# LouisNUST/pose-unsupervised

Measured on AMD Instinct MI355X. Metric: 4-view 256x256 frames/sec (fwd+triangulate), higher is better.
Workload: dtype bf16

## Files before the change

### pose-unsupervised_amd/csrc/stem.hip

```cpp
#include <string>
#include <type_traits>

#include "posu_common.h"

namespace posu {
namespace {

constexpr int kStemK = 224;
constexpr int kStemPitch = 232;
typedef unsigned int u32x4 __attribute__((ext_vector_type(4)));

template <typename T>
struct StemOp;
template <>
struct StemOp<uint16_t> {
  static __device__ __forceinline__ void mma(f32x4& acc, const uint4& a, const uint4& b) {
    acc = __builtin_amdgcn_mfma_f32_16x16x32_bf16(__builtin_bit_cast(bf16x8, a), __builtin_bit_cast(bf16x8, b), acc,
                                                  0, 0, 0);
  }
  static __device__ __forceinline__ uint32_t pack2(float a, float b) {
    return f2bf2(a, b);
  }
};
template <>
struct StemOp<f16_t> {
  static __device__ __forceinline__ void mma(f32x4& acc, const uint4& a, const uint4& b) {
    acc = __builtin_amdgcn_mfma_f32_16x16x32_f16(__builtin_bit_cast(f16x8, a), __builtin_bit_cast(f16x8, b), acc, 0,
                                                 0, 0);
  }
  static __device__ __forceinline__ uint32_t pack2(float a, float b) {
    const _Float16 ha = static_cast<_Float16>(a), hb = static_cast<_Float16>(b);
    return static_cast<uint32_t>(__builtin_bit_cast(uint16_t, ha)) |
           (static_cast<uint32_t>(__builtin_bit_cast(uint16_t, hb)) << 16);
  }
};

constexpr int kMaxViews = 8;
struct StemViews {
  const float* x[kMaxViews];
};

#ifndef POSU_STEM_ABLATE
#define POSU_STEM_ABLATE 0
#endif
#ifndef POSU_STEM_PFD
#define POSU_STEM_PFD 1
#endif
constexpr int kStemAbl = POSU_STEM_ABLATE;

template <typename T, int NW, bool SPL = false, bool RAW = false>
__global__ __launch_bounds__(NW * 64, 1) void stem_pool_kernel(StemViews xs, int Nv, int N, int H, int W, int hflip,
                                                               int strips, const void* __restrict__ wv_,
                                                               const float* __restrict__ scale,
                                                               const float* __restrict__ shift, T* __restrict__ y) {
  using O = StemOp<T>;
  constexpr int NT = NW * 64;
  constexpr int WP = NW * 32 + 8;
  constexpr int RB = WP * 8;
  constexpr int RING = 16;
  constexpr int W_BYTES = 64 * kStemPitch * 2;
  constexpr int NS = SPL ? 2 : 1;
  constexpr int CPX = SPL ? 128 : 64;
  static_assert(!SPL || (NW == 8 && std::is_same<T, f16_t>::value), "split stem: fp16 halves, eight waves");
  static_assert(!RAW || (!SPL && NW == 8), "raw stem: one dtype, eight waves");
  const T* __restrict__ w = static_cast<const T*>(wv_);
  __shared__ __attribute__((aligned(16))) char smem[NS * (RING * RB + W_BYTES) + NW * 2 * 64 * 4 + 2 * 64 * 4];
  char* win = smem;
  char* winl = smem + RING * RB;
  char* wl = smem + NS * RING * RB;
  char* wll = wl + W_BYTES;
  float* edge = reinterpret_cast<float*>(smem + NS * (RING * RB + W_BYTES));
  float* bn = edge + NW * 2 * 64;

  const int tid = threadIdx.x, lane = tid & 63, wid = tid >> 6;
  const int r16 = lane & 15, q = lane >> 4;
  const int Hp = H / 4, Wp = W / 4;
  const int pairs = Hp / 2, per = pairs / strips;
  const int n = blockIdx.x / strips;
  const int k0 = (blockIdx.x - n * strips) * per, k1 = k0 + per;
  const float* __restrict__ xn = xs.x[n / Nv] + static_cast<size_t>(n % Nv) * 3 * H * W;
  const size_t plane = static_cast<size_t>(H) * W;

  if constexpr (RAW) {
    const float* __restrict__ wf = static_cast<const float*>(wv_);
    for (int i = tid; i < 64 * kStemK / 2; i += NT) {
      const int co = i / (kStemK / 2), k0 = 2 * (i - co * (kStemK / 2));
      float v[2];
#pragma unroll
      for (int u = 0; u < 2; ++u) {
        const int k = k0 + u, kh = k >> 5, kw = (k >> 2) & 7, ci = k & 3;
        v[u] = (kw < 7 && ci < 3) ? wf[((co * 3 + ci) * 7 + kh) * 7 + kw] : 0.f;
      }
      *reinterpret_cast<uint32_t*>(wl + (co * kStemPitch + k0) * 2) = O::pack2(v[0], v[1]);
    }
  } else {
  if (tid < 64) {
    bn[tid] = fabsf(scale[tid]);
    bn[64 + tid] = shift[tid];
  }
  {
    constexpr int WCH = 64 * (kStemK / 8);
#pragma unroll
    for (int it = 0; it < (NS * WCH + NT - 1) / NT; ++it) {
      const int i = tid + it * NT;
      if (i < NS * WCH) {
        const int h = i / WCH, ii = i - h * WCH;
        const int co = ii / (kStemK / 8), ck = ii - co * (kStemK / 8);
        const unsigned sg = __float_as_uint(scale[co]) & 0x80000000u ? 0x80008000u : 0u;
        u32x4 wv = *reinterpret_cast<const u32x4*>(w + i * 8);
        wv ^= sg;
        *reinterpret_cast<u32x4*>((h ? wll : wl) + (co * kStemPitch + ck * 8) * 2) = wv;
      }
    }
  }
  }

  constexpr int GPR = NW * 8 + 2;
  constexpr int XG8 = (8 * GPR + NT - 1) / NT;
  auto load_rows = [&](int i0, auto nr, float4 (*xv)[3]) __attribute__((always_inline)) {
    constexpr int NR = decltype(nr)::value, XG = (NR * GPR + NT - 1) / NT;
#pragma unroll
    for (int it = 0; it < XG; ++it) {
      const int i = tid + it * NT;
      const int r = i / GPR, gk = i - r * GPR;
      const int iy = i0 + r, c0 = 4 * (gk - 1);
#pragma unroll
      for (int p = 0; p < 3; ++p) xv[it][p] = make_float4(0.f, 0.f, 0.f, 0.f);
      if (kStemAbl & 2) {
        xv[it][0] = make_float4(iy, c0, 1.f, 0.5f);
        continue;
      }
      if (i < NR * GPR && static_cast<unsigned>(iy) < static_cast<unsigned>(H) &&
          static_cast<unsigned>(c0) < static_cast<unsigned>(W)) {
        const size_t o = static_cast<size_t>(iy) * W + (hflip ? W - 4 - c0 : c0);
#pragma unroll
        for (int p = 0; p < 3; ++p) {
          float4 v = *reinterpret_cast<const float4*>(xn + p * plane + o);
          if (hflip) v = make_float4(v.w, v.z, v.y, v.x);
          xv[it][p] = v;
        }
      }
    }
  };
  auto store_rows = [&](int i0, auto nr, float4 (*xv)[3]) __attribute__((always_inline)) {
    constexpr int NR = decltype(nr)::value, XG = (NR * GPR + NT - 1) / NT;
#pragma unroll
    for (int it = 0; it < XG; ++it) {
      const int i = tid + it * NT;
      if (i >= NR * GPR) continue;
      const int r = i / GPR, gk = i - r * GPR;
      char* row = win + ((i0 + r) & (RING - 1)) * RB;
      const float a0[4] = {xv[it][0].x, xv[it][0].y, xv[it][0].z, xv[it][0].w};
      const float a1[4] = {xv[it][1].x, xv[it][1].y, xv[it][1].z, xv[it][1].w};
      const float a2[4] = {xv[it][2].x, xv[it][2].y, xv[it][2].z, xv[it][2].w};
#pragma unroll
      for (int e = 0; e < 4; ++e) {
        const int wc = 4 * gk - 1 + e;
        if (wc >= 0 && wc < WP) {
          *reinterpret_cast<uint2*>(row + wc * 8) = make_uint2(O::pack2(a0[e], a1[e]), O::pack2(a2[e], 0.f));
          if constexpr (SPL) {
            const float l0 = a0[e] - static_cast<float>(static_cast<_Float16>(a0[e]));
            const float l1 = a1[e] - static_cast<float>(static_cast<_Float16>(a1[e]));
            const float l2 = a2[e] - static_cast<float>(static_cast<_Float16>(a2[e]));
            *reinterpret_cast<uint2*>(row - win + winl + wc * 8) = make_uint2(O::pack2(l0, l1), O::pack2(l2, 0.f));
          }
        }
      }
    }
  };

  const int sc = 16 * wid + r16;
  auto stem_rows = [&](int r0, auto mrows, float (*carry)[4], float (*vm)[4][4]) __attribute__((always_inline)) {
    constexpr int M = decltype(mrows)::value;
    f32x4 acc[M][4];
#pragma unroll
    for (int i = 0; i < M; ++i)
#pragma unroll
      for (int j = 0; j < 4; ++j) acc[i][j] = f32x4{0.f, 0.f, 0.f, 0.f};
    auto rd = [&](int rho) {
      return *reinterpret_cast<const uint4*>(win + ((2 * r0 - 3 + rho) & (RING - 1)) * RB + (2 * sc + 2 * q) * 8);
    };
    auto rdl = [&](int rho) {
      return *reinterpret_cast<const uint4*>(winl + ((2 * r0 - 3 + rho) & (RING - 1)) * RB + (2 * sc + 2 * q) * 8);
    };
    auto bload = [&](int kh, uint4 (&bfr)[4]) {
#pragma unroll
      for (int j = 0; j < 4; ++j)
        bfr[j] = *reinterpret_cast<const uint4*>(wl + ((16 * j + r16) * kStemPitch + kh * 32 + 8 * q) * 2);
    };
    auto bloadl = [&](int kh, uint4 (&bfr)[4]) {
#pragma unroll
      for (int j = 0; j < 4; ++j)
        bfr[j] = *reinterpret_cast<const uint4*>(wll + ((16 * j + r16) * kStemPitch + kh * 32 + 8 * q) * 2);
    };
    auto mmas = [&](const uint4 (&bfr)[4], const uint4 (&af)[M]) {
#pragma unroll
      for (int rl = 0; rl < M; ++rl)
#pragma unroll
        for (int j = 0; j < 4; ++j) {
          if (kStemAbl & 1) acc[rl][j][0] += __uint_as_float(bfr[j].x ^ af[rl].y);
          else O::mma(acc[rl][j], bfr[j], af[rl]);
        }
    };
    if constexpr (SPL) {
      uint4 ev[M], od[M], evl[M], odl[M], bfr[4], bfl[4];
#pragma unroll
      for (int kh = 0; kh < 7; ++kh) {
        uint4 (&set)[M] = (kh & 1) ? od : ev;
        uint4 (&setl)[M] = (kh & 1) ? odl : evl;
        bload(kh, bfr);
        bloadl(kh, bfl);
        if (kh < 2) {
#pragma unroll
          for (int rl = 0; rl < M; ++rl) {
            set[rl] = rd(kh + 2 * rl);
            setl[rl] = rdl(kh + 2 * rl);
          }
        } else {
#pragma unroll
          for (int rl = 0; rl + 1 < M; ++rl) {
            set[rl] = set[rl + 1];
            setl[rl] = setl[rl + 1];
          }
          set[M - 1] = rd(kh + 2 * (M - 1));
          setl[M - 1] = rdl(kh + 2 * (M - 1));
        }
        mmas(bfr, set);
        mmas(bfl, set);
        mmas(bfr, setl);
      }
    } else if constexpr (NW <= 8) {
      uint4 ev[M], od[M], bfr[4];
#pragma unroll
      for (int kh = 0; kh < 7; ++kh) {
        uint4 (&set)[M] = (kh & 1) ? od : ev;
        bload(kh, bfr);
        if (kh < 2) {
#pragma unroll
          for (int rl = 0; rl < M; ++rl) set[rl] = rd(kh + 2 * rl);
        } else {
#pragma unroll
          for (int rl = 0; rl + 1 < M; ++rl) set[rl] = set[rl + 1];
          set[M - 1] = rd(kh + 2 * (M - 1));
        }
        mmas(bfr, set);
      }
    } else {
#pragma unroll 1
      for (int kh = 0; kh < 7; ++kh) {
        uint4 bfr[4];
        bload(kh, bfr);
#pragma unroll
        for (int rl = 0; rl < M; ++rl) {
          const uint4 af = rd(kh + 2 * rl);
#pragma unroll
          for (int j = 0; j < 4; ++j) O::mma(acc[rl][j], bfr[j], af);
        }
      }
    }
    if constexpr (RAW) {
      T* __restrict__ zr = y + (static_cast<size_t>(n) * (H / 2) + r0) * (W / 2) * 64 + sc * 64 + 4 * q;
#pragma unroll
      for (int rl = 0; rl < M; ++rl)
#pragma unroll
        for (int j = 0; j < 4; ++j) {
          const uint2 u = make_uint2(O::pack2(acc[rl][j][0], acc[rl][j][1]), O::pack2(acc[rl][j][2], acc[rl][j][3]));
          if (kStemAbl & 4) asm volatile("" ::"v"(u.x), "v"(u.y));
          else *reinterpret_cast<uint2*>(zr + static_cast<size_t>(rl) * (W / 2) * 64 + 16 * j) = u;
        }
      return;
    }
#pragma unroll
    for (int j = 0; j < 4; ++j)
#pragma unroll
      for (int e = 0; e < 4; ++e) {
        float v[M];
#pragma unroll
        for (int rl = 0; rl < M; ++rl)
          v[rl] = (M == 4 || r0 + rl >= 0) ? acc[rl][j][e] : -INFINITY;
        const float first = M == 5 ? v[0] : carry[j][e];
        const float* u = v + (M == 5 ? 1 : 0);
        vm[0][j][e] = fmaxf(fmaxf(first, u[0]), u[1]);
        vm[1][j][e] = fmaxf(fmaxf(u[1], u[2]), u[3]);
        carry[j][e] = u[3];
      }
  };

  T* __restrict__ yn = y + static_cast<size_t>(n) * Hp * Wp * CPX;
  auto pool = [&](int k, const float (*vm)[4][4]) __attribute__((always_inline)) {
    if (r16 == 15) {
#pragma unroll
      for (int p = 0; p < 2; ++p)
#pragma unroll
        for (int j = 0; j < 4; ++j)
          *reinterpret_cast<float4*>(edge + (wid * 2 + p) * 64 + 16 * j + 4 * q) =
              make_float4(vm[p][j][0], vm[p][j][1], vm[p][j][2], vm[p][j][3]);
    }
    __syncthreads();
    const int wl = wid > 0 ? wid - 1 : 0;
    const bool first_col = r16 == 0, pad_left = wid == 0;
#pragma unroll
    for (int p = 0; p < 2; ++p)
#pragma unroll
      for (int j = 0; j < 4; ++j) {
        const float4 s4 = *reinterpret_cast<const float4*>(bn + 16 * j + 4 * q);
        const float4 b4 = *reinterpret_cast<const float4*>(bn + 64 + 16 * j + 4 * q);
        const float sv[4] = {s4.x, s4.y, s4.z, s4.w}, bv[4] = {b4.x, b4.y, b4.z, b4.w};
        const float4 l4 = *reinterpret_cast<const float4*>(edge + (wl * 2 + p) * 64 + 16 * j + 4 * q);
        const float lv[4] = {l4.x, l4.y, l4.z, l4.w};
        float o[4];
#pragma unroll
        for (int e = 0; e < 4; ++e) {
          const float self = vm[p][j][e];
          const float right = __int_as_float(__builtin_amdgcn_update_dpp(0, __float_as_int(self), 0x101, 0xf, 0xf, true));
          float left = __int_as_float(__builtin_amdgcn_update_dpp(0, __float_as_int(self), 0x111, 0xf, 0xf, true));
          if (first_col) left = pad_left ? -INFINITY : lv[e];
          o[e] = fmaxf(fmaf(sv[e], fmaxf(fmaxf(left, self), right), bv[e]), 0.f);
        }
        if ((r16 & 1) == 0) {
          const int pc = 8 * wid + (r16 >> 1);
          const int c0 = 16 * j + 4 * q;
          T* dst = yn + (static_cast<size_t>(2 * k + p) * Wp + pc) * CPX + (SPL ? split_ch(c0) : c0);
          const uint2 u = make_uint2(O::pack2(o[0], o[1]), O::pack2(o[2], o[3]));
          if (kStemAbl & 4) {
            asm volatile("" ::"v"(u.x), "v"(u.y));
          } else {
            *reinterpret_cast<uint2*>(dst) = u;
            if constexpr (SPL) {
              float l[4];
#pragma unroll
              for (int e = 0; e < 4; ++e) l[e] = o[e] - static_cast<float>(static_cast<_Float16>(o[e]));
              *reinterpret_cast<uint2*>(dst + 32) = make_uint2(O::pack2(l[0], l[1]), O::pack2(l[2], l[3]));
            }
          }
        }
      }
  };

  using I4 = std::integral_constant<int, 4>;
  using I5 = std::integral_constant<int, 5>;
  using I8 = std::integral_constant<int, 8>;
  float carry[4][4], vm[2][4][4];
  constexpr bool PF = NW <= 8;
  constexpr int PFD = PF ? POSU_STEM_PFD : 1;
  static_assert(PFD == 1 || PFD == 2, "prefetch depth 1 or 2");
  float4 xv[PFD][XG8][3];
  load_rows(8 * k0 - 5, I8{}, xv[0]);
  store_rows(8 * k0 - 5, I8{}, xv[0]);
  load_rows(8 * k0 + 3, I8{}, xv[0]);
  store_rows(8 * k0 + 3, I8{}, xv[0]);
  __syncthreads();
  if constexpr (RAW) stem_rows(4 * k0, I4{}, carry, vm);
  else stem_rows(4 * k0 - 1, I5{}, carry, vm);
  if constexpr (PF) {
    if (k0 + 1 < k1) load_rows(8 * k0 + 10, I8{}, xv[PFD - 1]);
    if (PFD == 2 && k0 + 2 < k1) load_rows(8 * k0 + 18, I8{}, xv[0]);
  }
  if constexpr (RAW) __syncthreads();
  else pool(k0, vm);
  auto item = [&](int k, auto sidx) __attribute__((always_inline)) {
    constexpr int S = decltype(sidx)::value;
    if (!PF) load_rows(8 * k + 2, I8{}, xv[S]);
    store_rows(8 * k + 2, I8{}, xv[S]);
    __syncthreads();
    if (PF && k + PFD < k1) load_rows(8 * (k + PFD) + 2, I8{}, xv[S]);
    if constexpr (PF) stem_rows(4 * k, I4{}, carry, vm);
    else stem_rows(4 * k - 1, I5{}, carry, vm);
    if constexpr (RAW) {
      __syncthreads();
    } else {
      pool(k, vm);
    }
  };
  using S0 = std::integral_constant<int, 0>;
  using S1 = std::integral_constant<int, PFD - 1>;
  int k = k0 + 1;
  if constexpr (PFD == 2) {
    for (; k + 1 < k1; k += 2) {
      item(k, S1{});
      item(k + 1, S0{});
    }
  }
  for (; k < k1; ++k) item(k, S1{});
}


typedef short s16x4 __attribute__((ext_vector_type(4)));
constexpr int kWgThreads = 448;
constexpr int kWgRing = 16;
constexpr int kWgCols = 264;
constexpr int kWgRB = kWgCols * 8;
constexpr int kWgDz = 128 * 128;
constexpr int kWgGroups = 66;
constexpr int kWgPart = 7 * 32 * 64;

__device__ __forceinline__ int wg_sw(int px) { return (((px >> 1) & 1) << 1) | (((px >> 3) & 1) << 2); }

__device__ __forceinline__ uint4 tr_pair(const char* p0, const char* p1) {
  const s16x4 v0 = __builtin_amdgcn_ds_read_tr16_b64_v4i16((__attribute__((address_space(3))) s16x4*)(p0));
  const s16x4 v1 = __builtin_amdgcn_ds_read_tr16_b64_v4i16((__attribute__((address_space(3))) s16x4*)(p1));
  const uint2 u0 = __builtin_bit_cast(uint2, v0), u1 = __builtin_bit_cast(uint2, v1);
  return make_uint4(u0.x, u0.y, u1.x, u1.y);
}

template <typename T>
__global__ __launch_bounds__(kWgThreads, 2) void stem_wgrad_kernel(StemViews xs, int Nv, int H, int strips,
                                                                   const T* __restrict__ dz, float* __restrict__ part) {
  using O = StemOp<T>;
  constexpr int W = 256, Wo = 128;
  __shared__ __attribute__((aligned(16))) char smem[kWgRing * kWgRB + 2 * kWgDz];
  char* ring = smem;
  char* dzb = smem + kWgRing * kWgRB;
  const int tid = threadIdx.x, lane = tid & 63, kh = tid >> 6;
  const int q = lane >> 4, a = (lane >> 2) & 3, p = lane & 3;
  const int Ho = H / 2, rows = Ho / strips;
  const int n = blockIdx.x / strips;
  const int ya = (blockIdx.x - n * strips) * rows, yb = ya + rows;
  const float* __restrict__ xn = xs.x[n / Nv] + static_cast<size_t>(n % Nv) * 3 * H * W;
  const size_t plane = static_cast<size_t>(H) * W;
  const T* __restrict__ dzn = dz + static_cast<size_t>(n) * Ho * Wo * 64;

  auto load_x = [&](int iy0, int nr, int it, float4 (&xv)[3]) {
    const int i = tid + it * kWgThreads;
    const int r = i / kWgGroups, g = i - r * kWgGroups;
    const int iy = iy0 + r, c0 = 4 * (g - 1);
    const bool ok = i < nr * kWgGroups && static_cast<unsigned>(iy) < static_cast<unsigned>(H) &&
                    static_cast<unsigned>(c0) < static_cast<unsigned>(W);
    const size_t o = ok ? static_cast<size_t>(iy) * W + c0 : 0;
#pragma unroll
    for (int pl = 0; pl < 3; ++pl) {
      const float4 v = *reinterpret_cast<const float4*>(xn + pl * plane + o);
      xv[pl] = ok ? v : make_float4(0.f, 0.f, 0.f, 0.f);
    }
  };
  auto store_x = [&](int iy0, int nr, int it, const float4 (&xv)[3]) {
    const int i = tid + it * kWgThreads;
    if (i >= nr * kWgGroups) return;
    const int r = i / kWgGroups, g = i - r * kWgGroups;
    char* row = ring + ((iy0 + r) & (kWgRing - 1)) * kWgRB;
    auto cmp = [](const float4& v, int e) { return e == 0 ? v.x : e == 1 ? v.y : e == 2 ? v.z : v.w; };
#pragma unroll
    for (int e = 0; e < 4; ++e) {
      const int wc = 4 * g - 1 + e;
      if (wc >= 0 && wc < kWgCols)
        *reinterpret_cast<uint2*>(row + wc * 8) =
            make_uint2(O::pack2(cmp(xv[0], e), cmp(xv[1], e)), O::pack2(cmp(xv[2], e), 0.f));
    }
  };
  auto load_dz = [&](int oy, uint4 (&dv)[3]) {
#pragma unroll
    for (int it = 0; it < 3; ++it) {
      const int i = tid + it * kWgThreads;
      dv[it] = i < 1024 ? *reinterpret_cast<const uint4*>(dzn + (static_cast<size_t>(oy) * Wo) * 64 + i * 8)
                        : make_uint4(0, 0, 0, 0);
    }
  };
  auto store_dz = [&](int buf, const uint4 (&dv)[3]) {
#pragma unroll
    for (int it = 0; it < 3; ++it) {
      const int i = tid + it * kWgThreads;
      if (i < 1024) {
        const int px = i >> 3, c = i & 7;
        *reinterpret_cast<uint4*>(dzb + buf * kWgDz + px * 128 + ((c ^ wg_sw(px)) << 4)) = dv[it];
      }
    }
  };

  {
    float4 xv[3];
#pragma unroll
    for (int it = 0; it < (7 * kWgGroups + kWgThreads - 1) / kWgThreads; ++it) {
      load_x(2 * ya - 3, 7, it, xv);
      store_x(2 * ya - 3, 7, it, xv);
    }
    uint4 dv[3];
    load_dz(ya, dv);
    store_dz(0, dv);
  }
  __syncthreads();

  f32x4 acc[4][2];
#pragma unroll
  for (int mt = 0; mt < 4; ++mt)
#pragma unroll
    for (int hf = 0; hf < 2; ++hf) acc[mt][hf] = f32x4{0.f, 0.f, 0.f, 0.f};
  for (int oy = ya; oy < yb; ++oy) {
    const bool more = oy + 1 < yb;
    float4 xv[3];
    uint4 dv[3];
    if (more) {
      load_x(2 * oy + 4, 2, 0, xv);
      load_dz(oy + 1, dv);
    }
    const char* dzr = dzb + (oy & 1) * kWgDz;
    const char* xr = ring + ((2 * oy - 3 + kh) & (kWgRing - 1)) * kWgRB;
#pragma unroll
    for (int s = 0; s < 4; ++s) {
      const int px0 = 32 * s + 8 * q + a, px1 = px0 + 4;
      uint4 af[4], bf[2];
#pragma unroll
      for (int mt = 0; mt < 4; ++mt) {
        const int chunk = 2 * mt + (p >> 1), within = (p & 1) * 8;
        af[mt] = tr_pair(dzr + px0 * 128 + ((chunk ^ wg_sw(px0)) << 4) + within,
                         dzr + px1 * 128 + ((chunk ^ wg_sw(px1)) << 4) + within);
      }
#pragma unroll
      for (int hf = 0; hf < 2; ++hf)
        bf[hf] = tr_pair(xr + 16 * px0 + 32 * hf + 8 * p, xr + 16 * px1 + 32 * hf + 8 * p);
#pragma unroll
      for (int mt = 0; mt < 4; ++mt)
#pragma unroll
        for (int hf = 0; hf < 2; ++hf) {
          if (kStemAbl & 1) acc[mt][hf][0] += __uint_as_float(af[mt].x ^ bf[hf].y);
          else O::mma(acc[mt][hf], af[mt], bf[hf]);
        }
    }
    if (more) {
      store_x(2 * oy + 4, 2, 0, xv);
      store_dz((oy + 1) & 1, dv);
    }
    __syncthreads();
  }
  float* dst = part + static_cast<size_t>(blockIdx.x) * kWgPart + kh * 32 * 64;
#pragma unroll
  for (int mt = 0; mt < 4; ++mt)
#pragma unroll
    for (int hf = 0; hf < 2; ++hf)
      *reinterpret_cast<float4*>(dst + (16 * hf + (lane & 15)) * 64 + 16 * mt + 4 * q) =
          make_float4(acc[mt][hf][0], acc[mt][hf][1], acc[mt][hf][2], acc[mt][hf][3]);
}

constexpr int kWrLanes = 16;
__global__ __launch_bounds__(256) void stem_wgrad_reduce_kernel(const float* __restrict__ part, int nblocks,
                                                                 float* __restrict__ dw) {
  __shared__ float red[kWrLanes][17];
  const int c = threadIdx.x & 15, sl = threadIdx.x >> 4;
  const int rest = blockIdx.x >> 2, co = (blockIdx.x & 3) * 16 + c;
  const int ci = rest % 3, tap = rest / 3, kh = tap / 7, kw = tap - 7 * kh;
  const float* p = part + (kh * 32 + kw * 4 + ci) * 64 + co;
  float s = 0.f;
#pragma unroll 4
  for (int b = sl; b < nblocks; b += kWrLanes) s += p[static_cast<size_t>(b) * kWgPart];
  red[sl][c] = s;
  __syncthreads();
  if (threadIdx.x < 16) {
    float t = 0.f;
#pragma unroll
    for (int l = 0; l < kWrLanes; ++l) t += red[l][threadIdx.x];
    dw[((co * 3 + ci) * 7 + kh) * 7 + kw] = t;
  }
}

}
}

using namespace posu;

namespace {
int stem_launch(int dtype, const float* const* views, int nviews, int Nv, int H, int W, int hflip, const void* w,
                const float* scale, const float* shift, void* y, void* stream, const char* what) {
  const std::string wh(what);
  POSU_REQUIRE(dtype == POSU_BF16 || dtype == POSU_F16 || dtype == POSU_F16X3, wh + ": dtype must be BF16, F16 or F16X3");
  POSU_REQUIRE(dtype != POSU_F16X3 || W == 256, wh + ": the split-fp16 stem is built for W = 256");
  POSU_REQUIRE(views && nviews >= 1 && nviews <= kMaxViews, wh + ": 1 .. 8 views");
  for (int v = 0; v < nviews; ++v) POSU_REQUIRE(views[v], wh + ": null view pointer");
  POSU_REQUIRE(w && scale && shift && y, wh + ": null pointer");
  POSU_REQUIRE(Nv > 0 && H > 0 && H % 8 == 0 && (W == 256 || W == 384),
               wh + ": needs H % 8 == 0 and W in {256, 384}");
  POSU_REQUIRE(static_cast<long long>(Nv) * 3 * H * W < (1LL << 40), wh + ": input too large");
  StemViews xs{};
  for (int v = 0; v < nviews; ++v) xs.x[v] = views[v];
  const int N = Nv * nviews, pairs = H / 8;
  int strips = 1;
  while (N * strips * 2 <= 256 && pairs % (strips * 2) == 0) strips *= 2;
  hipStream_t s = as_stream(stream);
  const dim3 grid(static_cast<unsigned>(N * strips));
  if (dtype == POSU_F16X3) {
    hipLaunchKernelGGL((stem_pool_kernel<f16_t, 8, true>), grid, dim3(512), 0, s, xs, Nv, N, H, W, hflip, strips,
                       static_cast<const f16_t*>(w), scale, shift, static_cast<f16_t*>(y));
  } else if (dtype == POSU_BF16) {
    if (W == 256)
      hipLaunchKernelGGL((stem_pool_kernel<uint16_t, 8>), grid, dim3(512), 0, s, xs, Nv, N, H, W, hflip, strips,
                         static_cast<const uint16_t*>(w), scale, shift, static_cast<uint16_t*>(y));
    else
      hipLaunchKernelGGL((stem_pool_kernel<uint16_t, 12>), grid, dim3(768), 0, s, xs, Nv, N, H, W, hflip, strips,
                         static_cast<const uint16_t*>(w), scale, shift, static_cast<uint16_t*>(y));
  } else {
    if (W == 256)
      hipLaunchKernelGGL((stem_pool_kernel<f16_t, 8>), grid, dim3(512), 0, s, xs, Nv, N, H, W, hflip, strips,
                         static_cast<const f16_t*>(w), scale, shift, static_cast<f16_t*>(y));
    else
      hipLaunchKernelGGL((stem_pool_kernel<f16_t, 12>), grid, dim3(768), 0, s, xs, Nv, N, H, W, hflip, strips,
                         static_cast<const f16_t*>(w), scale, shift, static_cast<f16_t*>(y));
  }
  return check_launch(what);
}
}

extern "C" int posu_stem_pool_fwd(int dtype, const float* x, int N, int H, int W, int hflip, const void* w,
                                  const float* scale, const float* shift, void* y, void* stream) {
  return stem_launch(dtype, &x, 1, N, H, W, hflip, w, scale, shift, y, stream, "posu_stem_pool_fwd");
}

extern "C" int posu_stem_pool_views_fwd(int dtype, const float* const* views, int nviews, int Nv, int H, int W,
                                        int hflip, const void* w, const float* scale, const float* shift, void* y,
                                        void* stream) {
  return stem_launch(dtype, views, nviews, Nv, H, W, hflip, w, scale, shift, y, stream, "posu_stem_pool_views_fwd");
}

namespace {
int stem_train_views(const char* what, int dtype, const float* const* views, int nviews, int Nv, int H, int W,
                     StemViews& xs) {
  const std::string wh(what);
  POSU_REQUIRE(dtype == POSU_BF16 || dtype == POSU_F16, wh + ": dtype must be BF16 or F16");
  POSU_REQUIRE(views && nviews >= 1 && nviews <= kMaxViews, wh + ": 1 .. 8 views");
  for (int v = 0; v < nviews; ++v) POSU_REQUIRE(views[v], wh + ": null view pointer");
  POSU_REQUIRE(Nv > 0 && H > 0 && H % 8 == 0 && W == 256, wh + ": built for W = 256 and H % 8 == 0");
  POSU_REQUIRE(static_cast<long long>(Nv) * 3 * H * W < (1LL << 40), wh + ": input too large");
  for (int v = 0; v < nviews; ++v) {
    POSU_REQUIRE((reinterpret_cast<size_t>(views[v]) & 15) == 0, wh + ": views must be 16-byte aligned");
    xs.x[v] = views[v];
  }
  return 0;
}

int wgrad_strips(int N, int H) {
  int strips = 1;
  while (N * strips * 2 <= 512 && (H / 2) % (strips * 2) == 0 && (H / 2) / (strips * 2) >= 8) strips *= 2;
  return strips;
}
}

extern "C" int posu_stem_conv_views_fwd(int dtype, const float* const* views, int nviews, int Nv, int H, int W,
                                        const float* w, void* z, void* stream) {
  StemViews xs{};
  const int rc = stem_train_views("posu_stem_conv_views_fwd", dtype, views, nviews, Nv, H, W, xs);
  if (rc) return rc;
  POSU_REQUIRE(w && z, "posu_stem_conv_views_fwd: null pointer");
  const int N = Nv * nviews, pairs = H / 8;
  int strips = 1;
  while (N * strips * 2 <= 256 && pairs % (strips * 2) == 0) strips *= 2;
  hipStream_t s = as_stream(stream);
  const dim3 grid(static_cast<unsigned>(N * strips));
  if (dtype == POSU_BF16)
    hipLaunchKernelGGL((stem_pool_kernel<uint16_t, 8, false, true>), grid, dim3(512), 0, s, xs, Nv, N, H, W, 0, strips,
                       static_cast<const void*>(w), nullptr, nullptr, static_cast<uint16_t*>(z));
  else
    hipLaunchKernelGGL((stem_pool_kernel<f16_t, 8, false, true>), grid, dim3(512), 0, s, xs, Nv, N, H, W, 0, strips,
                       static_cast<const void*>(w), nullptr, nullptr, static_cast<f16_t*>(z));
  return check_launch("posu_stem_conv_views_fwd");
}

extern "C" long long posu_stem_wgrad_workspace(int N, int H, int W) {
  if (N <= 0 || H <= 0 || H % 8 != 0 || W != 256) return -1;
  return static_cast<long long>(N) * wgrad_strips(N, H) * kWgPart * 4;
}

extern "C" int posu_stem_wgrad_views(int dtype, const float* const* views, int nviews, int Nv, int H, int W,
                                     const void* dz, float* dw, void* workspace, long long workspace_bytes,
                                     void* stream) {
  StemViews xs{};
  const int rc = stem_train_views("posu_stem_wgrad_views", dtype, views, nviews, Nv, H, W, xs);
  if (rc) return rc;
  POSU_REQUIRE(dz && dw && workspace, "posu_stem_wgrad_views: null pointer");
  POSU_REQUIRE((reinterpret_cast<size_t>(dz) & 15) == 0 && (reinterpret_cast<size_t>(workspace) & 15) == 0,
               "posu_stem_wgrad_views: dz / workspace must be 16-byte aligned");
  const int N = Nv * nviews, strips = wgrad_strips(N, H);
  POSU_REQUIRE(workspace_bytes >= posu_stem_wgrad_workspace(N, H, W), "posu_stem_wgrad_views: workspace too small");
  hipStream_t s = as_stream(stream);
  float* part = static_cast<float*>(workspace);
  const dim3 grid(static_cast<unsigned>(N * strips));
  if (dtype == POSU_BF16)
    hipLaunchKernelGGL(stem_wgrad_kernel<uint16_t>, grid, dim3(kWgThreads), 0, s, xs, Nv, H, strips,
                       static_cast<const uint16_t*>(dz), part);
  else
    hipLaunchKernelGGL(stem_wgrad_kernel<f16_t>, grid, dim3(kWgThreads), 0, s, xs, Nv, H, strips,
                       static_cast<const f16_t*>(dz), part);
  hipLaunchKernelGGL(stem_wgrad_reduce_kernel, dim3(147 * 4), dim3(256), 0, s, part, N * strips, dw);
  return check_launch("posu_stem_wgrad_views");
}
```

Before: 54010.

## Pipeline stem pooling into next strip's MFMA loop with buffer loads

Adds a pipelined path for the 8-wave non-split stem kernel: the ring grows to 32 rows, edge scratch is double-buffered, and the pool/BN/ReLU/store of the previous strip is interleaved between kernel-row MFMA steps of the next strip, removing one barrier per strip. Global input loads and output stores switch to raw buffer loads and stores, with out-of-range offsets replacing explicit bounds branches. Padding columns are zero-filled once so each thread handles exactly one column group. This costs more LDS and register pressure, and the interleaving may disturb the MFMA schedule.

```diff
diff --git a/pose-unsupervised_amd/csrc/stem.hip b/pose-unsupervised_amd/csrc/stem.hip
--- a/pose-unsupervised_amd/csrc/stem.hip
+++ b/pose-unsupervised_amd/csrc/stem.hip
@@ -1,11 +1,12 @@
 #include <string>
 #include <type_traits>
 
-#include "posu_common.h"
+#include "gemm_common.h"
 
 namespace posu {
 namespace {
 
+typedef unsigned int u32x2 __attribute__((ext_vector_type(2)));
 constexpr int kStemK = 224;
 constexpr int kStemPitch = 232;
 typedef unsigned int u32x4 __attribute__((ext_vector_type(4)));
@@ -47,6 +48,9 @@
 #define POSU_STEM_PFD 1
 #endif
 constexpr int kStemAbl = POSU_STEM_ABLATE;
+#ifndef POSU_STEM_PIPE
+#define POSU_STEM_PIPE 1
+#endif
 
 template <typename T, int NW, bool SPL = false, bool RAW = false>
 __global__ __launch_bounds__(NW * 64, 1) void stem_pool_kernel(StemViews xs, int Nv, int N, int H, int W, int hflip,
@@ -57,20 +61,23 @@
   constexpr int NT = NW * 64;
   constexpr int WP = NW * 32 + 8;
   constexpr int RB = WP * 8;
-  constexpr int RING = 16;
+  constexpr bool PIPE = NW == 8 && !SPL && !RAW && POSU_STEM_PIPE;
+  constexpr int RING = PIPE ? 32 : 16;
+  constexpr int NE = PIPE ? 2 : 1;
   constexpr int W_BYTES = 64 * kStemPitch * 2;
   constexpr int NS = SPL ? 2 : 1;
   constexpr int CPX = SPL ? 128 : 64;
   static_assert(!SPL || (NW == 8 && std::is_same<T, f16_t>::value), "split stem: fp16 halves, eight waves");
   static_assert(!RAW || (!SPL && NW == 8), "raw stem: one dtype, eight waves");
   const T* __restrict__ w = static_cast<const T*>(wv_);
-  __shared__ __attribute__((aligned(16))) char smem[NS * (RING * RB + W_BYTES) + NW * 2 * 64 * 4 + 2 * 64 * 4];
+  constexpr int EW = NW + 1;
+  __shared__ __attribute__((aligned(16))) char smem[NS * (RING * RB + W_BYTES) + NE * EW * 2 * 64 * 4 + 2 * 64 * 4];
   char* win = smem;
   char* winl = smem + RING * RB;
   char* wl = smem + NS * RING * RB;
   char* wll = wl + W_BYTES;
   float* edge = reinterpret_cast<float*>(smem + NS * (RING * RB + W_BYTES));
-  float* bn = edge + NW * 2 * 64;
+  float* bn = edge + NE * EW * 2 * 64;
 
   const int tid = threadIdx.x, lane = tid & 63, wid = tid >> 6;
   const int r16 = lane & 15, q = lane >> 4;
@@ -79,7 +86,8 @@
   const int n = blockIdx.x / strips;
   const int k0 = (blockIdx.x - n * strips) * per, k1 = k0 + per;
   const float* __restrict__ xn = xs.x[n / Nv] + static_cast<size_t>(n % Nv) * 3 * H * W;
-  const size_t plane = static_cast<size_t>(H) * W;
+  const unsigned plane4 = static_cast<unsigned>(H) * W * 4u;
+  const __amdgpu_buffer_rsrc_t xrs = __builtin_amdgcn_make_buffer_rsrc(const_cast<float*>(xn), 0, 3 * H * W * 4, 0x00020000);
 
   if constexpr (RAW) {
     const float* __restrict__ wf = static_cast<const float*>(wv_);
@@ -98,6 +106,7 @@
     bn[tid] = fabsf(scale[tid]);
     bn[64 + tid] = shift[tid];
   }
+  if (tid < NE * 128) edge[(tid >> 7) * EW * 128 + (tid & 127)] = -INFINITY;
   {
     constexpr int WCH = 64 * (kStemK / 8);
 #pragma unroll
@@ -115,62 +124,55 @@
   }
   }
 
-  constexpr int GPR = NW * 8 + 2;
-  constexpr int XG8 = (8 * GPR + NT - 1) / NT;
+  if (tid < RING * 8) {
+    const int c = tid & 7, off = (tid >> 3) * RB + (c < 3 ? c : WP - 8 + c) * 8;
+    *reinterpret_cast<uint2*>(win + off) = make_uint2(0u, 0u);
+    if constexpr (SPL) *reinterpret_cast<uint2*>(winl + off) = make_uint2(0u, 0u);
+  }
+  constexpr int GPR = NW * 8;
+  constexpr int XG8 = 1;
+  static_assert(8 * GPR == NT, "8 rows = one column group per thread");
+  const int xr = tid / GPR, xg = tid - xr * GPR;
   auto load_rows = [&](int i0, auto nr, float4 (*xv)[3]) __attribute__((always_inline)) {
-    constexpr int NR = decltype(nr)::value, XG = (NR * GPR + NT - 1) / NT;
-#pragma unroll
-    for (int it = 0; it < XG; ++it) {
-      const int i = tid + it * NT;
-      const int r = i / GPR, gk = i - r * GPR;
-      const int iy = i0 + r, c0 = 4 * (gk - 1);
-#pragma unroll
-      for (int p = 0; p < 3; ++p) xv[it][p] = make_float4(0.f, 0.f, 0.f, 0.f);
-      if (kStemAbl & 2) {
-        xv[it][0] = make_float4(iy, c0, 1.f, 0.5f);
-        continue;
-      }
-      if (i < NR * GPR && static_cast<unsigned>(iy) < static_cast<unsigned>(H) &&
-          static_cast<unsigned>(c0) < static_cast<unsigned>(W)) {
-        const size_t o = static_cast<size_t>(iy) * W + (hflip ? W - 4 - c0 : c0);
-#pragma unroll
-        for (int p = 0; p < 3; ++p) {
-          float4 v = *reinterpret_cast<const float4*>(xn + p * plane + o);
-          if (hflip) v = make_float4(v.w, v.z, v.y, v.x);
-          xv[it][p] = v;
-        }
-      }
+    static_assert(decltype(nr)::value == 8, "8 rows at a time");
+    const int iy = i0 + xr, c0 = 4 * xg;
+    if (kStemAbl & 2) {
+#pragma unroll
+      for (int p = 0; p < 3; ++p) xv[0][p] = make_float4(0.f, 0.f, 0.f, 0.f);
+      xv[0][0] = make_float4(iy, c0, 1.f, 0.5f);
+      return;
+    }
+    const bool ok = static_cast<unsigned>(iy) < static_cast<unsigned>(H);
+    const unsigned o = ok ? static_cast<unsigned>(iy * W + (hflip ? W - 4 - c0 : c0)) * 4u : static_cast<unsigned>(kOOB);
+#pragma unroll
+    for (int p = 0; p < 3; ++p) {
+      float4 v = __builtin_bit_cast(float4, __builtin_amdgcn_raw_buffer_load_b128(xrs, o + p * plane4, 0, 0));
+      if (hflip) v = make_float4(v.w, v.z, v.y, v.x);
+      xv[0][p] = v;
     }
   };
   auto store_rows = [&](int i0, auto nr, float4 (*xv)[3]) __attribute__((always_inline)) {
-    constexpr int NR = decltype(nr)::value, XG = (NR * GPR + NT - 1) / NT;
-#pragma unroll
-    for (int it = 0; it < XG; ++it) {
-      const int i = tid + it * NT;
-      if (i >= NR * GPR) continue;
-      const int r = i / GPR, gk = i - r * GPR;
-      char* row = win + ((i0 + r) & (RING - 1)) * RB;
-      const float a0[4] = {xv[it][0].x, xv[it][0].y, xv[it][0].z, xv[it][0].w};
-      const float a1[4] = {xv[it][1].x, xv[it][1].y, xv[it][1].z, xv[it][1].w};
-      const float a2[4] = {xv[it][2].x, xv[it][2].y, xv[it][2].z, xv[it][2].w};
-#pragma unroll
-      for (int e = 0; e < 4; ++e) {
-        const int wc = 4 * gk - 1 + e;
-        if (wc >= 0 && wc < WP) {
-          *reinterpret_cast<uint2*>(row + wc * 8) = make_uint2(O::pack2(a0[e], a1[e]), O::pack2(a2[e], 0.f));
-          if constexpr (SPL) {
-            const float l0 = a0[e] - static_cast<float>(static_cast<_Float16>(a0[e]));
-            const float l1 = a1[e] - static_cast<float>(static_cast<_Float16>(a1[e]));
-            const float l2 = a2[e] - static_cast<float>(static_cast<_Float16>(a2[e]));
-            *reinterpret_cast<uint2*>(row - win + winl + wc * 8) = make_uint2(O::pack2(l0, l1), O::pack2(l2, 0.f));
-          }
-        }
+    static_assert(decltype(nr)::value == 8, "8 rows at a time");
+    char* row = win + ((i0 + xr) & (RING - 1)) * RB;
+    const float a0[4] = {xv[0][0].x, xv[0][0].y, xv[0][0].z, xv[0][0].w};
+    const float a1[4] = {xv[0][1].x, xv[0][1].y, xv[0][1].z, xv[0][1].w};
+    const float a2[4] = {xv[0][2].x, xv[0][2].y, xv[0][2].z, xv[0][2].w};
+#pragma unroll
+    for (int e = 0; e < 4; ++e) {
+      const int wc = 4 * xg + 3 + e;
+      *reinterpret_cast<uint2*>(row + wc * 8) = make_uint2(O::pack2(a0[e], a1[e]), O::pack2(a2[e], 0.f));
+      if constexpr (SPL) {
+        const float l0 = a0[e] - static_cast<float>(static_cast<_Float16>(a0[e]));
+        const float l1 = a1[e] - static_cast<float>(static_cast<_Float16>(a1[e]));
+        const float l2 = a2[e] - static_cast<float>(static_cast<_Float16>(a2[e]));
+        *reinterpret_cast<uint2*>(row - win + winl + wc * 8) = make_uint2(O::pack2(l0, l1), O::pack2(l2, 0.f));
       }
     }
   };
 
   const int sc = 16 * wid + r16;
-  auto stem_rows = [&](int r0, auto mrows, float (*carry)[4], float (*vm)[4][4]) __attribute__((always_inline)) {
+  auto stem_rows = [&](int r0, auto mrows, float (*carry)[4], float (*vm)[4][4], auto between)
+                       __attribute__((always_inline)) {
     constexpr int M = decltype(mrows)::value;
     f32x4 acc[M][4];
 #pragma unroll
@@ -234,7 +236,7 @@
 #pragma unroll
       for (int kh = 0; kh < 7; ++kh) {
         uint4 (&set)[M] = (kh & 1) ? od : ev;
-        bload(kh, bfr);
+        if (!(kStemAbl & 8) || kh == 0) bload(kh, bfr);
         if (kh < 2) {
 #pragma unroll
           for (int rl = 0; rl < M; ++rl) set[rl] = rd(kh + 2 * rl);
@@ -244,6 +246,7 @@
           set[M - 1] = rd(kh + 2 * (M - 1));
         }
         mmas(bfr, set);
+        between(kh);
       }
     } else {
 #pragma unroll 1
@@ -287,55 +290,60 @@
   };
 
   T* __restrict__ yn = y + static_cast<size_t>(n) * Hp * Wp * CPX;
+  const __amdgpu_buffer_rsrc_t yrs =
+      __builtin_amdgcn_make_buffer_rsrc(RAW ? y : yn, 0, RAW ? 0 : Hp * Wp * CPX * 2, 0x00020000);
+  const unsigned pool_off = (r16 & 1) ? static_cast<unsigned>(kOOB) : (8 * wid + (r16 >> 1)) * CPX * 2;
+  auto edge_write = [&](int eb, const float (*vm)[4][4]) __attribute__((always_inline)) {
+    if (r16 == 15) {
+#pragma unroll
+      for (int p = 0; p < 2; ++p)
+#pragma unroll
+        for (int j = 0; j < 4; ++j)
+          *reinterpret_cast<float4*>(edge + ((eb * EW + wid + 1) * 2 + p) * 64 + 16 * j + 4 * q) =
+              make_float4(vm[p][j][0], vm[p][j][1], vm[p][j][2], vm[p][j][3]);
+    }
+  };
+  auto pool_tile = [&](int k, int eb, const float (*vm)[4][4], int j) __attribute__((always_inline)) {
+    const float4 s4 = *reinterpret_cast<const float4*>(bn + 16 * j + 4 * q);
+    const float4 b4 = *reinterpret_cast<const float4*>(bn + 64 + 16 * j + 4 * q);
+    const float sv[4] = {s4.x, s4.y, s4.z, s4.w}, bv[4] = {b4.x, b4.y, b4.z, b4.w};
+#pragma unroll
+    for (int p = 0; p < 2; ++p) {
+      const float4 l4 = *reinterpret_cast<const float4*>(edge + ((eb * EW + wid) * 2 + p) * 64 + 16 * j + 4 * q);
+      const float lv[4] = {l4.x, l4.y, l4.z, l4.w};
+      float o[4];
+#pragma unroll
+      for (int e = 0; e < 4; ++e) {
+        const float self = vm[p][j][e];
+        const float right = __int_as_float(__builtin_amdgcn_update_dpp(0, __float_as_int(self), 0x101, 0xf, 0xf, true));
+        const float left = __int_as_float(
+            __builtin_amdgcn_update_dpp(__float_as_int(lv[e]), __float_as_int(self), 0x111, 0xf, 0xf, false));
+        o[e] = fmaxf(fmaf(sv[e], fmaxf(fmaxf(left, self), right), bv[e]), 0.f);
+      }
+      const int c0 = 16 * j + 4 * q;
+      const unsigned off = pool_off + static_cast<unsigned>(((2 * k + p) * Wp * CPX + (SPL ? split_ch(c0) : c0)) * 2);
+      const u32x2 u = {O::pack2(o[0], o[1]), O::pack2(o[2], o[3])};
+      if (kStemAbl & 4) {
+        asm volatile("" ::"v"(u.x), "v"(u.y));
+      } else {
+        __builtin_amdgcn_raw_buffer_store_b64(u, yrs, off, 0, 0);
+        if constexpr (SPL) {
+          float l[4];
+#pragma unroll
+          for (int e = 0; e < 4; ++e) l[e] = o[e] - static_cast<float>(static_cast<_Float16>(o[e]));
+          const u32x2 ul = {O::pack2(l[0], l[1]), O::pack2(l[2], l[3])};
+          __builtin_amdgcn_raw_buffer_store_b64(ul, yrs, off + 64, 0, 0);
+        }
+      }
+    }
+  };
   auto pool = [&](int k, const float (*vm)[4][4]) __attribute__((always_inline)) {
-    if (r16 == 15) {
-#pragma unroll
-      for (int p = 0; p < 2; ++p)
-#pragma unroll
-        for (int j = 0; j < 4; ++j)
-          *reinterpret_cast<float4*>(edge + (wid * 2 + p) * 64 + 16 * j + 4 * q) =
-              make_float4(vm[p][j][0], vm[p][j][1], vm[p][j][2], vm[p][j][3]);
-    }
+    edge_write(0, vm);
     __syncthreads();
-    const int wl = wid > 0 ? wid - 1 : 0;
-    const bool first_col = r16 == 0, pad_left = wid == 0;
-#pragma unroll
-    for (int p = 0; p < 2; ++p)
-#pragma unroll
-      for (int j = 0; j < 4; ++j) {
-        const float4 s4 = *reinterpret_cast<const float4*>(bn + 16 * j + 4 * q);
-        const float4 b4 = *reinterpret_cast<const float4*>(bn + 64 + 16 * j + 4 * q);
-        const float sv[4] = {s4.x, s4.y, s4.z, s4.w}, bv[4] = {b4.x, b4.y, b4.z, b4.w};
-        const float4 l4 = *reinterpret_cast<const float4*>(edge + (wl * 2 + p) * 64 + 16 * j + 4 * q);
-        const float lv[4] = {l4.x, l4.y, l4.z, l4.w};
-        float o[4];
-#pragma unroll
-        for (int e = 0; e < 4; ++e) {
-          const float self = vm[p][j][e];
-          const float right = __int_as_float(__builtin_amdgcn_update_dpp(0, __float_as_int(self), 0x101, 0xf, 0xf, true));
-          float left = __int_as_float(__builtin_amdgcn_update_dpp(0, __float_as_int(self), 0x111, 0xf, 0xf, true));
-          if (first_col) left = pad_left ? -INFINITY : lv[e];
-          o[e] = fmaxf(fmaf(sv[e], fmaxf(fmaxf(left, self), right), bv[e]), 0.f);
-        }
-        if ((r16 & 1) == 0) {
-          const int pc = 8 * wid + (r16 >> 1);
-          const int c0 = 16 * j + 4 * q;
-          T* dst = yn + (static_cast<size_t>(2 * k + p) * Wp + pc) * CPX + (SPL ? split_ch(c0) : c0);
-          const uint2 u = make_uint2(O::pack2(o[0], o[1]), O::pack2(o[2], o[3]));
-          if (kStemAbl & 4) {
-            asm volatile("" ::"v"(u.x), "v"(u.y));
-          } else {
-            *reinterpret_cast<uint2*>(dst) = u;
-            if constexpr (SPL) {
-              float l[4];
-#pragma unroll
-              for (int e = 0; e < 4; ++e) l[e] = o[e] - static_cast<float>(static_cast<_Float16>(o[e]));
-              *reinterpret_cast<uint2*>(dst + 32) = make_uint2(O::pack2(l[0], l[1]), O::pack2(l[2], l[3]));
-            }
-          }
-        }
-      }
-  };
+#pragma unroll
+    for (int j = 0; j < 4; ++j) pool_tile(k, 0, vm, j);
+  };
+  auto nothing = [](int) {};
 
   using I4 = std::integral_constant<int, 4>;
   using I5 = std::integral_constant<int, 5>;
@@ -350,8 +358,28 @@
   load_rows(8 * k0 + 3, I8{}, xv[0]);
   store_rows(8 * k0 + 3, I8{}, xv[0]);
   __syncthreads();
-  if constexpr (RAW) stem_rows(4 * k0, I4{}, carry, vm);
-  else stem_rows(4 * k0 - 1, I5{}, carry, vm);
+  if constexpr (PIPE) {
+    if (k0 + 1 < k1) load_rows(8 * k0 + 10, I8{}, xv[0]);
+    stem_rows(4 * k0 - 1, I5{}, carry, vm, nothing);
+    if (k0 + 1 < k1) store_rows(8 * k0 + 10, I8{}, xv[0]);
+    edge_write(k0 & 1, vm);
+    for (int k = k0 + 1; k < k1; ++k) {
+      if (!(kStemAbl & 16)) __syncthreads();
+      if (k + 1 < k1) load_rows(8 * k + 10, I8{}, xv[0]);
+      stem_rows(4 * k, I4{}, carry, vm, [&](int kh) __attribute__((always_inline)) {
+        if (kh == 1 || kh == 2) pool_tile(k - 1, (k - 1) & 1, vm, kh - 1);
+        if (kh == 4 || kh == 5) pool_tile(k - 1, (k - 1) & 1, vm, kh - 2);
+      });
+      if (k + 1 < k1) store_rows(8 * k + 10, I8{}, xv[0]);
+      edge_write(k & 1, vm);
+    }
+    __syncthreads();
+#pragma unroll
+    for (int j = 0; j < 4; ++j) pool_tile(k1 - 1, (k1 - 1) & 1, vm, j);
+    return;
+  }
+  if constexpr (RAW) stem_rows(4 * k0, I4{}, carry, vm, nothing);
+  else stem_rows(4 * k0 - 1, I5{}, carry, vm, nothing);
   if constexpr (PF) {
     if (k0 + 1 < k1) load_rows(8 * k0 + 10, I8{}, xv[PFD - 1]);
     if (PFD == 2 && k0 + 2 < k1) load_rows(8 * k0 + 18, I8{}, xv[0]);
@@ -364,8 +392,8 @@
     store_rows(8 * k + 2, I8{}, xv[S]);
     __syncthreads();
     if (PF && k + PFD < k1) load_rows(8 * (k + PFD) + 2, I8{}, xv[S]);
-    if constexpr (PF) stem_rows(4 * k, I4{}, carry, vm);
-    else stem_rows(4 * k - 1, I5{}, carry, vm);
+    if constexpr (PF) stem_rows(4 * k, I4{}, carry, vm, nothing);
+    else stem_rows(4 * k - 1, I5{}, carry, vm, nothing);
     if constexpr (RAW) {
       __syncthreads();
     } else {
@@ -567,7 +595,8 @@
   POSU_REQUIRE(w && scale && shift && y, wh + ": null pointer");
   POSU_REQUIRE(Nv > 0 && H > 0 && H % 8 == 0 && (W == 256 || W == 384),
                wh + ": needs H % 8 == 0 and W in {256, 384}");
-  POSU_REQUIRE(static_cast<long long>(Nv) * 3 * H * W < (1LL << 40), wh + ": input too large");
+  POSU_REQUIRE(static_cast<long long>(Nv) * 3 * H * W < (1LL << 40) && H <= (1 << 16),
+               wh + ": input too large");
   StemViews xs{};
   for (int v = 0; v < nviews; ++v) xs.x[v] = views[v];
   const int N = Nv * nviews, pairs = H / 8;
@@ -616,7 +645,7 @@
   POSU_REQUIRE(views && nviews >= 1 && nviews <= kMaxViews, wh + ": 1 .. 8 views");
   for (int v = 0; v < nviews; ++v) POSU_REQUIRE(views[v], wh + ": null view pointer");
   POSU_REQUIRE(Nv > 0 && H > 0 && H % 8 == 0 && W == 256, wh + ": built for W = 256 and H % 8 == 0");
-  POSU_REQUIRE(static_cast<long long>(Nv) * 3 * H * W < (1LL << 40), wh + ": input too large");
+  POSU_REQUIRE(static_cast<long long>(Nv) * 3 * H * W < (1LL << 40) && H <= (1 << 16), wh + ": input too large");
   for (int v = 0; v < nviews; ++v) {
     POSU_REQUIRE((reinterpret_cast<size_t>(views[v]) & 15) == 0, wh + ": views must be 16-byte aligned");
     xs.x[v] = views[v];
```

Result: no change. 54260, median of 6 (+0.5%).
